# wildltr/ptranking

Measured on NVIDIA H100. Metric: queries/sec (LambdaRank train step, 256-doc lists), higher is better.
Workload: dtype f32

## Files before the change

ptranking_b200/csrc/ffnet_tc.cuh:

```cuda
#pragma once
#include "common.cuh"
#include "tc.cuh"
#include "ffnet_act.cuh"

namespace ptrb200 {

struct RowsGemmArgs {
    const float* P;
    const float* scale;
    const float* shift;
    int act;
    int gr_prev;
    DropCfg drop;
    const float* P2;
    const float *kc1, *kc3, *kc0;
    int gr_cur;
    const unsigned char* b_img_hi;
    const unsigned char* b_img_lo;
    const float* bias;
    float* a_out;
    float* Out;
    double* partials;
    int rows, K, N, NP;
    int n_tile;
// ... 558 lines not shown
    #pragma unroll
                    for (int i = 0; i < RW_PU; ++i) { cur[i] = pre[i]; cur2[i] = pre2[i]; }
                    if (q + 1 < total_q) {
                        if (c + 1 < nchunks) fetch(c + 1); else { point(it + 1); fetch(0); }
                    }
                    if (q >= 2) tc::mbar_wait(afree + s, ((q - 2) >> 1) & 1);
                    unsigned char* a_hi = a_ring + s * 32768;
                    if (partial && c == lastc) {
    #pragma unroll
                        for (int i = 0; i < RW_PU; ++i) {
                            const int jB = jB_[i];
                            if (jB < zfill) {
                                float4 v = make_float4(0.f, 0.f, 0.f, 0.f);
                                if (jB < vlast && rB < nrows) {
                                    const int col = lastc * 32 + jB * 4;
                                    const size_t e0 = (size_t)(row0 + rB) * K + col;
                                    const size_t co = (per_group ? (size_t)((row0 + rB) / g.gr_prev) * K : (size_t)0) + col;
                                    const size_t kc = ((fused_dz && g.gr_cur < g.rows) ? (size_t)((row0 + rB) / g.gr_cur) * K : (size_t)0) + col;
                                    v = xform(cur[i], cur2[i], has_coef ? g.scale + co : nullptr, has_coef ? g.shift + co : nullptr, kc,
                                              (uint64_t)e0 >> 2, (MODE == RG_FWD && g.a_out) ? g.a_out + e0 : nullptr);
                                }
                                store_split(a_hi, a_hi + 16384, tc::swz_offset(rB, jB), v, PASSES == 3, PASSES == 1 && g.round_bf16 != 0);
                            }
                        }
                    } else {
                        const bool kv = c * 32 + j4 < K;
    #pragma unroll
                        for (int i = 0; i < RW_PU; ++i) {
                            float4 v = make_float4(0.f, 0.f, 0.f, 0.f);
                            if (live[i] && kv)
                                v = xform(cur[i], cur2[i], has_coef ? sc[i] + c * 32 : nullptr, has_coef ? sh[i] + c * 32 : nullptr,
                                          kco[i] + c * 32, dq[i] + c * 8, aout[i] ? aout[i] + c * 32 : nullptr);
                            store_split(a_hi, a_hi + 16384, sw_[i], v, PASSES == 3, PASSES == 1 && g.round_bf16 != 0);
                        }
                    }
                    tc::fence_proxy_async();
                    __syncwarp();
                    if (lane == 0) tc::mbar_arrive(aready + s);
                }
            }
        }
    } else {
        tc::setmaxnreg_dec<RW_CONS_REGS>();
        if (my_tiles > 0) {
        const int wg = warp >> 2;
        if (tid == 0) {
            tc::mbar_expect_tx(wfull, (uint32_t)(nchunks * wchunk * (PASSES == 3 ? 2 : 1)));
            for (int c = 0; c < nchunks; ++c) {
                tc::bulk_g2s(w_hi + (size_t)c * wchunk, g.b_img_hi + (size_t)c * wchunk, wchunk, wfull);
                if (PASSES == 3) tc::bulk_g2s(w_lo + (size_t)c * wchunk, g.b_img_lo + (size_t)c * wchunk, wchunk, wfull);
            }
        }
        tc::mbar_wait(wfull, 0);
        const uint32_t a_base = tc::smem_u32(a_ring) + wg * 8192, wh_base = tc::smem_u32(w_hi), wl_base = tc::smem_u32(w_lo);
        double acc1 = 0.0, acc2 = 0.0;
        tc::with_width(NP, [&](auto W) {
        constexpr int NPc = decltype(W)::value;
        int q = 0;
        for (int it = 0; it < my_tiles; ++it) {
            const int t = blockIdx.x + it * gridDim.x;
            int row0, nrows;
            rw_tile(g, t, row0, nrows);
            float acc[NPc / 2];
#pragma unroll
            for (int e = 0; e < NPc / 2; ++e) acc[e] = 0.0f;
    #pragma unroll (KT ? 8 : 1)
            for (int c = 0; c < nchunks; ++c, ++q) {
                const int s = q & 1;
                tc::mbar_wait(aready + s, (q >> 1) & 1);
                uint32_t a_addr = a_base + s * 32768, b_off = c * wchunk;
                asm volatile("" : "+r"(a_addr), "+r"(b_off));
                const uint64_t ah = tc::smem_desc_sw128(a_addr, 1024), al = tc::smem_desc_sw128(a_addr + 16384, 1024);
                const uint64_t bh = tc::smem_desc_sw128(wh_base + b_off, 1024), bl = tc::smem_desc_sw128(wl_base + b_off, 1024);
                tc::wg_fence();
#pragma unroll
                for (int st = 0; st < 4; ++st) {
                    if (PASSES == 3) {
                        tc::mma_tf32<NPc>(acc, al + 2 * st, bh + 2 * st, 1u);
                        tc::mma_tf32<NPc>(acc, ah + 2 * st, bl + 2 * st, 1u);
                    }
                    tc::mma_tf32<NPc>(acc, ah + 2 * st, bh + 2 * st, 1u);
                }
                tc::wg_commit();
                tc::wg_wait<1>();
                if (c > 0) { __syncwarp(); if (lane == 0) tc::mbar_arrive(afree + (s ^ 1)); }
            }
            tc::wg_wait<0>();
            __syncwarp();
            if (lane == 0) tc::mbar_arrive(afree + ((q - 1) & 1));
            const float* bias = g.bias;
            asm volatile("" : "+l"(bias));
            bool live[2];
            float* orow[2];
#pragma unroll
            for (int h = 0; h < 2; ++h) {
                const int r = wg * 64 + tc::acc_row(2 * h);
                live[h] = r < nrows;
                orow[h] = g.Out + (size_t)(row0 + min(r, nrows - 1)) * N;
            }
            if (MODE == RG_FWD) {
#pragma unroll
                for (int e = 0; e < NPc / 2; ++e) {
                    const int col = tc::acc_col(e);
                    if (col >= N) { acc[e] = 0.0f; continue; }
                    acc[e] += __ldg(bias + col);
                }
            } else if (g.drop.thr && (N & 3) == 0) {
                const bool odd = lane & 1;
#pragma unroll
                for (int e = 0; e < NPc / 2; e += 4) {
                    const int col = tc::acc_col(e);
                    const uint64_t el = (uint64_t)(row0 + wg * 64 + tc::acc_row(e) + (odd ? 8 : 0)) * N + (col & ~3);
                    const uint64_t d = dropout_draw4(g.drop.key, el >> 2);
                    const uint32_t other = __shfl_xor_sync(0xffffffffu, odd ? (uint32_t)d : (uint32_t)(d >> 32), 1);
                    const uint32_t ur = odd ? other : (uint32_t)d;
                    const uint32_t ur8 = odd ? (uint32_t)(d >> 32) : other;
                    if (col >= N) { acc[e] = acc[e + 1] = acc[e + 2] = acc[e + 3] = 0.0f; continue; }
                    acc[e] = (ur & 0xffffu) >= g.drop.thr ? acc[e] * g.drop.scale : 0.0f;
                    acc[e + 1] = (ur >> 16) >= g.drop.thr ? acc[e + 1] * g.drop.scale : 0.0f;
                    acc[e + 2] = (ur8 & 0xffffu) >= g.drop.thr ? acc[e + 2] * g.drop.scale : 0.0f;
                    acc[e + 3] = (ur8 >> 16) >= g.drop.thr ? acc[e + 3] * g.drop.scale : 0.0f;
                }
            } else {
#pragma unroll
                for (int e = 0; e < NPc / 2; ++e) {
                    const int col = tc::acc_col(e);
                    if (col >= N) { acc[e] = 0.0f; continue; }
                    if (g.drop.thr) {
                        const int r = wg * 64 + tc::acc_row(e);
                        acc[e] = dropout_keep(g.drop.key, (uint64_t)(row0 + r) * N + col, g.drop.thr) ? acc[e] * g.drop.scale : 0.0f;
                    }
                }
            }
#pragma unroll
            for (int e = 0; e < NPc / 2; e += 2) {
                const int col = tc::acc_col(e), h = (e >> 1) & 1;
                if (!live[h] || col >= N) continue;
                if ((N & 1) == 0) *reinterpret_cast<float2*>(orow[h] + col) = make_float2(acc[e], acc[e + 1]);
                else { orow[h][col] = acc[e]; if (col + 1 < N) orow[h][col + 1] = acc[e + 1]; }
            }
            if (MODE == RG_FWD && x.stats_mode) {
                int sl = lane, sw = warp;
                asm volatile("" : "+r"(sl), "+r"(sw));
#pragma unroll
                for (int j = 0; j < NPc / 16; ++j) {
                    const float* w = acc + 8 * j;
                    float s[8];
#pragma unroll
                    for (int p = 0; p < 4; ++p) {
                        const int e0 = (p >> 1) * 4 + (p & 1), e1 = e0 + 2;
                        const float v0 = live[0] ? w[e0] : 0.0f, v1 = live[1] ? w[e1] : 0.0f;
                        s[p] = v0 + v1; s[4 + p] = v0 * v0 + v1 * v1;
                    }
#pragma unroll
                    for (int st = 0; st < 3; ++st) {
                        const int h = 4 >> st, o = 4 << st;
                        const bool up = sl & o;
#pragma unroll
                        for (int i = 0; i < h; ++i) {
                            float keep = s[i], send = s[i + h];
                            if (up) { const float t = keep; keep = send; send = t; }
                            s[i] = keep + __shfl_xor_sync(0xffffffffu, send, o);
                        }
                    }
                    const int v = ((sl >> 2) & 1) * 4 + ((sl >> 3) & 1) * 2 + ((sl >> 4) & 1), p = v & 3;
                    const int col = j * 16 + (p >> 1) * 8 + 2 * (sl & 3) + (p & 1);
                    stat_sm[(sw * NP + col) * 2 + (v >> 2)] = s[0];
                }
                asm volatile("bar.sync 2, 256;" ::: "memory");
                if (tid < N) {
                    double s1 = 0.0, s2 = 0.0;
#pragma unroll
                    for (int w = 0; w < RW_EPI_WARPS; ++w) { s1 += (double)stat_sm[(w * NP + tid) * 2]; s2 += (double)stat_sm[(w * NP + tid) * 2 + 1]; }
                    if (x.stats_mode == 2) {
                        double* p = g.partials + ((size_t)t * N + tid) * 2;
                        p[0] = s1; p[1] = s2;
                    } else { acc1 += s1; acc2 += s2; }
                }
                asm volatile("bar.sync 2, 256;" ::: "memory");
            }
        }
        });
        if (MODE == RG_FWD && x.stats_mode == 1 && tid < N) {
            double* p = g.partials + ((size_t)blockIdx.x * N + tid) * 2;
            p[0] = acc1; p[1] = acc2;
        }
        } else if (MODE == RG_FWD && x.stats_mode == 1 && tid < N) {
            double* p = g.partials + ((size_t)blockIdx.x * N + tid) * 2;
            p[0] = 0.0; p[1] = 0.0;
        }
    }
}

struct WgradArgs {
    const float* Z2;
    const float *kc1, *kc3, *kc0;
    int gr_cur;
    const float* dZ;
    const float* P;
    const float* scale;
    const float* shift;
    int act, gr_prev;
    DropCfg drop;
    float* partials;
    int rows, K, N;
    int KP;
    int N_full, K_full;
    int kb;
    int tile_rows;
    int stages;
    int round_bf16;
};

constexpr int WG_THREADS = 512;
constexpr int WG_MAX_STAGES = 4;

template <int PASSES, bool XB = false>
__global__ void __launch_bounds__(WG_THREADS, 1) wgrad_tc_kernel(WgradArgs g) {
    extern __shared__ __align__(1024) unsigned char smem_raw[];
    unsigned char* base = reinterpret_cast<unsigned char*>((reinterpret_cast<uintptr_t>(smem_raw) + 1023) & ~(uintptr_t)1023);
    const int R = g.tile_rows;
    const int m0 = blockIdx.y * 128, kk0 = blockIdx.z * g.kb;
    const int N = min(128, g.N_full - m0), K = min(g.kb, g.K_full - kk0), KP = ((K + 15) / 16) * 16;
    const int Nmax = min(128, g.N_full), Kmax = min(g.kb, g.K_full);
    const bool blocked = gridDim.y > 1 || gridDim.z > 1;
    const int KPmax = ((Kmax + 15) / 16) * 16;
    const int zop_bytes = 128 * 128, pop_bytes = KPmax * 128;
    const int op_bytes = (zop_bytes + pop_bytes) * (PASSES == 3 ? 2 : 1);
    const bool fused_dz = g.Z2 != nullptr;
    const int rawz1 = ((R * Nmax * 4 + 127) / 128) * 128;
    constexpr int PB = XB ? 2 : 4;
    const int rawz_bytes = rawz1 * (fused_dz ? 2 : 1), rawp_bytes = ((R * Kmax * PB + 127) / 128) * 128;
    const int stages = g.stages;
    unsigned char* opbuf = base;
    unsigned char* rawbuf = opbuf + 2 * op_bytes;
    unsigned char* tail = rawbuf + stages * (rawz_bytes + rawp_bytes);
    uint64_t* full = reinterpret_cast<uint64_t*>(tail);

    const int tid = threadIdx.x, warp = tid >> 5, lane = tid & 31, wg = warp >> 2;
    if (tid == 0) {
        for (int s = 0; s < stages; ++s) tc::mbar_init(full + s, 1);
        tc::mbar_fence_init();
    }
    const int ntiles = (g.rows + R - 1) / R;
    const int my_tiles = blockIdx.x < ntiles ? (ntiles - blockIdx.x + gridDim.x - 1) / gridDim.x : 0;

    bool p_bulk_ok = true;
    if constexpr (XB) p_bulk_ok = ((reinterpret_cast<uintptr_t>(g.P) & 15) == 0) && (!blocked || (K % 8 == 0 && g.K_full % 8 == 0));
    auto p_bulk = [&](int nrows) -> bool {
        if constexpr (XB) return p_bulk_ok && (blocked || (((uint32_t)nrows * K * 2) & 15) == 0);
        else return true;
    };

    auto issue_load = [&](int it, int s) {
        const int t = blockIdx.x + it * gridDim.x;
        const int row0 = t * R, nrows = min(R, g.rows - row0);
        const bool pbk = p_bulk(nrows);
        const uint32_t zb = (uint32_t)nrows * N * 4, pb = pbk ? (uint32_t)nrows * K * PB : 0u;
        unsigned char* rz = rawbuf + s * (rawz_bytes + rawp_bytes);
        if (!blocked) {
            if (lane == 0) {
                if ((zb & 15) == 0) {
                    tc::mbar_expect_tx(full + s, (fused_dz ? 2 * zb : zb) + pb);
                    tc::bulk_g2s(rz, g.dZ + (size_t)row0 * N, zb, full + s);
                    if (fused_dz) tc::bulk_g2s(rz + rawz1, g.Z2 + (size_t)row0 * N, zb, full + s);
                } else {
                    tc::mbar_expect_tx(full + s, pb);
                }
                if constexpr (XB) { if (pbk) tc::bulk_g2s(rz + rawz_bytes, reinterpret_cast<const uint16_t*>(g.P) + (size_t)row0 * K, pb, full + s); }
                else tc::bulk_g2s(rz + rawz_bytes, g.P + (size_t)row0 * K, pb, full + s);
            }
        } else {
            const bool z_bulk = (N & 3) == 0;
            if (lane == 0) tc::mbar_expect_tx(full + s, (z_bulk ? zb : 0u) + pb);
            __syncwarp();
            if (lane < nrows) {
                if (z_bulk) tc::bulk_g2s(rz + (size_t)lane * N * 4, g.dZ + (size_t)(row0 + lane) * g.N_full + m0, (uint32_t)N * 4, full + s);
                if constexpr (XB) {
                    if (pbk) tc::bulk_g2s(rz + rawz_bytes + (size_t)lane * K * 2, reinterpret_cast<const uint16_t*>(g.P) + (size_t)(row0 + lane) * g.K_full + kk0,
                                          (uint32_t)K * 2, full + s);
                } else tc::bulk_g2s(rz + rawz_bytes + (size_t)lane * K * 4, g.P + (size_t)(row0 + lane) * g.K_full + kk0, (uint32_t)K * 4, full + s);
            }
            __syncwarp();
        }
    };

    const bool plain_p = !g.scale && g.act == PTRB200_AF_NONE && !g.drop.thr;
    const bool single_group = fused_dz && g.gr_cur >= g.rows;
    float* coef = reinterpret_cast<float*>(tail + 128);
    {
        const uint32_t op_s = tc::smem_u32(opbuf);
        for (int e = tid; e < 2 * op_bytes / 16; e += WG_THREADS) tc::sts128(op_s + (uint32_t)e * 16u, make_float4(0.f, 0.f, 0.f, 0.f));
        if (single_group)
            for (int e = tid; e < 3 * 128; e += WG_THREADS) {
                const int which = e >> 7, n = e & 127;
                const float* src = which == 0 ? g.kc1 : which == 1 ? g.kc3 : g.kc0;
                coef[e] = n < N ? __ldg(src + m0 + n) : 0.0f;
            }
        __syncthreads();
    }
    if (warp == 0)
        for (int it = 0; it < min(stages, my_tiles); ++it) issue_load(it, it);

    auto put = [&](unsigned char* hi, unsigned char* lo, uint32_t off, float4 v) {
        if (PASSES == 3) {
            float4 h, l;
            tc::split_tf32(v.x, h.x, l.x); tc::split_tf32(v.y, h.y, l.y); tc::split_tf32(v.z, h.z, l.z); tc::split_tf32(v.w, h.w, l.w);
            *reinterpret_cast<float4*>(hi + off) = h;
            *reinterpret_cast<float4*>(lo + off) = l;
        } else {
            if (g.round_bf16) v = make_float4(bf16_rn(v.x), bf16_rn(v.y), bf16_rn(v.z), bf16_rn(v.w));
            *reinterpret_cast<float4*>(hi + off) = v;
        }
    };
    const int mh = wg & 1, KPh = ((KP / 16 + 1) / 2) * 16, c0 = (wg >> 1) ? KP - KPh : 0, cw0 = (wg >> 1) ? KPh : 0;
    const int RQ = R / 4;

    tc::with_width(KPh, [&](auto W) {
    constexpr int NPc = decltype(W)::value;
    float acc[NPc / 2];
#pragma unroll
    for (int e = 0; e < NPc / 2; ++e) acc[e] = 0.0f;
    for (int it = 0; it < my_tiles; ++it) {
        const int t = blockIdx.x + it * gridDim.x, o = it & 1, s = it % stages;
        const int row0 = t * R, nrows = min(R, g.rows - row0);
        const float* rz = reinterpret_cast<const float*>(rawbuf + s * (rawz_bytes + rawp_bytes));
        const float* rp = reinterpret_cast<const float*>(rawbuf + s * (rawz_bytes + rawp_bytes) + rawz_bytes);
        if (blocked ? (N & 3) != 0 : (((uint32_t)nrows * N * 4) & 15) != 0) {
            float* rzw = const_cast<float*>(rz);
            for (int e = tid; e < nrows * N; e += WG_THREADS) rzw[e] = g.dZ[(size_t)(row0 + e / N) * g.N_full + m0 + e % N];
            __syncthreads();
        }
        if constexpr (XB) {
            if (!p_bulk(nrows)) {
                uint16_t* rpw = reinterpret_cast<uint16_t*>(rawbuf + s * (rawz_bytes + rawp_bytes) + rawz_bytes);
                const uint16_t* src = reinterpret_cast<const uint16_t*>(g.P);
                for (int e = tid; e < nrows * K; e += WG_THREADS) rpw[e] = src[(size_t)(row0 + e / K) * g.K_full + kk0 + e % K];
                __syncthreads();
            }
        }
        tc::mbar_wait(full + s, (it / stages) & 1);
        unsigned char* zh = opbuf + o * op_bytes;
        unsigned char* zl = zh + zop_bytes;
        unsigned char* ph = zh + (PASSES == 3 ? 2 : 1) * zop_bytes;
        unsigned char* pl = ph + pop_bytes;
        for (int u = tid; u < 128 * RQ; u += WG_THREADS) {
            const int n = u & 127, qq = u >> 7;
            if (n >= N) continue;
            float v[4];
            const size_t grp_off_base = (size_t)m0 + n;
#pragma unroll
            for (int e = 0; e < 4; ++e) {
                const int r = qq * 4 + e;
                float x = 0.0f;
                if (r < nrows) {
                    x = rz[r * N + n];
                    if (fused_dz) {
                        const float z = rz[rawz1 / 4 + r * N + n];
                        float a1, a3, a0;
                        if (single_group) { a1 = coef[n]; a3 = coef[128 + n]; a0 = coef[256 + n]; }
                        else {
                            const size_t go = (size_t)((row0 + r) / g.gr_cur) * g.N_full + grp_off_base;
                            a1 = __ldg(g.kc1 + go); a3 = __ldg(g.kc3 + go); a0 = __ldg(g.kc0 + go);
                        }
                        x = fmaf(a1, x, fmaf(a3, z, a0));
                    }
                }
                v[e] = x;
            }
            put(zh, zl, tc::swz_offset(n, qq), make_float4(v[0], v[1], v[2], v[3]));
        }
        for (int u = tid; u < KP * RQ; u += WG_THREADS) {
            const int k = u % KP, qq = u / KP;
            if (k >= K) continue;
            float v[4];
#pragma unroll
            for (int e = 0; e < 4; ++e) {
                const int r = qq * 4 + e;
                float x = 0.0f;
                if (r < nrows) {
                    if constexpr (XB) x = __uint_as_float((uint32_t)reinterpret_cast<const uint16_t*>(rp)[r * K + k] << 16);
                    else x = rp[r * K + k];
                    if (!plain_p) {
                        const int row = row0 + r, col = kk0 + k;
                        if (g.scale) {
                            const size_t co = (g.gr_prev < g.rows ? (size_t)(row / g.gr_prev) * g.K_full : 0) + col;
                            x = fmaf(x, __ldg(g.scale + co), __ldg(g.shift + co));
                        }
                        if (g.act != PTRB200_AF_NONE) x = activate(g.act, x).y;
                        if (g.drop.thr) x = dropout_keep(g.drop.key, (uint64_t)row * g.K_full + col, g.drop.thr) ? x * g.drop.scale : 0.0f;
                    }
                }
                v[e] = x;
            }
            put(ph, pl, tc::swz_offset(k, qq), make_float4(v[0], v[1], v[2], v[3]));
        }
        tc::fence_proxy_async();
        __syncthreads();
        if (warp == 0 && it + stages < my_tiles) issue_load(it + stages, s);
        const uint32_t a_s = tc::smem_u32(zh) + mh * 8192, b_s = tc::smem_u32(ph) + c0 * 128;
        const uint64_t ah = tc::smem_desc_sw128(a_s, 1024), bh = tc::smem_desc_sw128(b_s, 1024);
        const uint64_t al = tc::smem_desc_sw128(a_s + zop_bytes, 1024), bl = tc::smem_desc_sw128(b_s + pop_bytes, 1024);
        tc::wg_fence();
#pragma unroll
        for (int st = 0; st < 4; ++st) {
            if (PASSES == 3) {
                tc::mma_tf32<NPc>(acc, al + 2 * st, bh + 2 * st, 1u);
                tc::mma_tf32<NPc>(acc, ah + 2 * st, bl + 2 * st, 1u);
            }
            tc::mma_tf32<NPc>(acc, ah + 2 * st, bh + 2 * st, 1u);
        }
        tc::wg_commit();
        tc::wg_wait<0>();
    }
    float* dst = g.partials + (size_t)blockIdx.x * g.N_full * g.K_full + (size_t)m0 * g.K_full + kk0;
#pragma unroll
    for (int e = 0; e < NPc / 2; ++e) {
        const int n = mh * 64 + tc::acc_row(e), k = c0 + tc::acc_col(e);
        if (n < N && k >= cw0 && k < K) dst[(size_t)n * g.K_full + k] = acc[e];
    }
    });
}

}
```

ptranking_b200/csrc/tc.cuh:

```cuda
#pragma once
#include <cuda_runtime.h>
#include <stdint.h>

namespace ptrb200 {
namespace tc {

template <int N> struct WidthT { static constexpr int value = N; };

constexpr int CHUNK_BYTES = 128;
constexpr int ATOM_BYTES = 1024;

__device__ __forceinline__ uint32_t smem_u32(const void* p) { return (uint32_t)__cvta_generic_to_shared(p); }

__device__ __forceinline__ uint32_t swz_offset(int r, int j) {
    return (uint32_t)((r >> 3) * ATOM_BYTES + (r & 7) * CHUNK_BYTES + ((j ^ (r & 7)) << 4));
}

__device__ __forceinline__ float4 lds128(uint32_t addr) {
    float4 v;
    asm volatile("ld.shared.v4.f32 {%0,%1,%2,%3}, [%4];" : "=f"(v.x), "=f"(v.y), "=f"(v.z), "=f"(v.w) : "r"(addr) : "memory");
    return v;
}
__device__ __forceinline__ float lds32(uint32_t addr) {
    float v;
    asm volatile("ld.shared.f32 %0, [%1];" : "=f"(v) : "r"(addr) : "memory");
    return v;
}
__device__ __forceinline__ void sts128(uint32_t addr, float4 v) {
    asm volatile("st.shared.v4.f32 [%0], {%1,%2,%3,%4};" ::"r"(addr), "f"(v.x), "f"(v.y), "f"(v.z), "f"(v.w) : "memory");
}

__device__ __forceinline__ void mbar_init(uint64_t* bar, uint32_t count) {
    asm volatile("mbarrier.init.shared::cta.b64 [%0], %1;" ::"r"(smem_u32(bar)), "r"(count) : "memory");
}
__device__ __forceinline__ void mbar_fence_init() { asm volatile("fence.mbarrier_init.release.cluster;" ::: "memory"); }
__device__ __forceinline__ void mbar_arrive(uint64_t* bar) {
    asm volatile("{\n\t.reg .b64 st;\n\tmbarrier.arrive.shared::cta.b64 st, [%0];\n\t}" ::"r"(smem_u32(bar)) : "memory");
}
__device__ __forceinline__ void mbar_expect_tx(uint64_t* bar, uint32_t bytes) {
    asm volatile("{\n\t.reg .b64 st;\n\tmbarrier.arrive.expect_tx.shared::cta.b64 st, [%0], %1;\n\t}" ::"r"(smem_u32(bar)), "r"(bytes) : "memory");
}
__device__ __forceinline__ bool mbar_try_wait(uint64_t* bar, uint32_t parity) {
    uint32_t ok;
    asm volatile(
        "{\n\t.reg .pred p;\n\t"
        "mbarrier.try_wait.parity.shared::cta.b64 p, [%1], %2;\n\t"
        "selp.u32 %0, 1, 0, p;\n\t}"
        : "=r"(ok) : "r"(smem_u32(bar)), "r"(parity) : "memory");
    return ok != 0;
}
__device__ __forceinline__ void mbar_wait(uint64_t* bar, uint32_t parity) {
    while (!mbar_try_wait(bar, parity)) {}
}
__device__ __forceinline__ void mbar_wait_relaxed(uint64_t* bar, uint32_t parity) {
    while (!mbar_try_wait(bar, parity)) { __nanosleep(40); }
}
__device__ __forceinline__ void fence_proxy_async() { asm volatile("fence.proxy.async.shared::cta;" ::: "memory"); }

template <int N>
__device__ __forceinline__ void setmaxnreg_dec() { asm volatile("setmaxnreg.dec.sync.aligned.u32 %0;" ::"n"(N)); }
template <int N>
__device__ __forceinline__ void setmaxnreg_inc() { asm volatile("setmaxnreg.inc.sync.aligned.u32 %0;" ::"n"(N)); }

__device__ __forceinline__ void bulk_g2s(void* smem_dst, const void* gmem_src, uint32_t bytes, uint64_t* bar) {
    asm volatile("cp.async.bulk.shared::cluster.global.mbarrier::complete_tx::bytes [%0], [%1], %2, [%3];"
                 ::"r"(smem_u32(smem_dst)), "l"(gmem_src), "r"(bytes), "r"(smem_u32(bar)) : "memory");
}
__device__ __forceinline__ void bulk_s2g(void* gmem_dst, const void* smem_src, uint32_t bytes) {
    asm volatile("cp.async.bulk.global.shared::cta.bulk_group [%0], [%1], %2;"
                 ::"l"(gmem_dst), "r"(smem_u32(smem_src)), "r"(bytes) : "memory");
}
__device__ __forceinline__ void bulk_commit() { asm volatile("cp.async.bulk.commit_group;" ::: "memory"); }
template <int N>
__device__ __forceinline__ void bulk_wait_read() { asm volatile("cp.async.bulk.wait_group.read %0;" ::"n"(N) : "memory"); }
template <int N>
__device__ __forceinline__ void bulk_wait() { asm volatile("cp.async.bulk.wait_group %0;" ::"n"(N) : "memory"); }

__device__ __forceinline__ uint64_t smem_desc_sw128(uint32_t smem_addr, uint32_t sbo_bytes) {
    uint64_t d = 0;
    d |= (uint64_t)((smem_addr & 0x3ffffu) >> 4);
    d |= (uint64_t)1 << 16;
    d |= (uint64_t)((sbo_bytes >> 4) & 0x3fffu) << 32;
    d |= (uint64_t)1 << 62;
    return d;
}

__device__ __forceinline__ void wg_fence() { asm volatile("wgmma.fence.sync.aligned;" ::: "memory"); }
__device__ __forceinline__ void wg_commit() { asm volatile("wgmma.commit_group.sync.aligned;" ::: "memory"); }
template <int N>
__device__ __forceinline__ void wg_wait() { asm volatile("wgmma.wait_group.sync.aligned %0;" ::"n"(N) : "memory"); }

template <int N>
__device__ __forceinline__ void mma_tf32(float (&d)[N / 2], uint64_t a_desc, uint64_t b_desc, uint32_t scale_d);

template <>
__device__ __forceinline__ void mma_tf32<16>(float (&d)[8], uint64_t a_desc, uint64_t b_desc, uint32_t scale_d) {
    asm volatile(
        "{\n\t.reg .pred p;\n\tsetp.ne.b32 p, %10, 0;\n\t"
        "wgmma.mma_async.sync.aligned.m64n16k8.f32.tf32.tf32 {%0,%1,%2,%3,%4,%5,%6,%7}, %8, %9, p, 1, 1;\n\t}"
        : "+f"(d[0]), "+f"(d[1]), "+f"(d[2]), "+f"(d[3]), "+f"(d[4]), "+f"(d[5]), "+f"(d[6]), "+f"(d[7])
        : "l"(a_desc), "l"(b_desc), "r"(scale_d) : "memory");
}

template <>
__device__ __forceinline__ void mma_tf32<32>(float (&d)[16], uint64_t a_desc, uint64_t b_desc, uint32_t scale_d) {
    asm volatile(
        "{\n\t.reg .pred p;\n\tsetp.ne.b32 p, %18, 0;\n\t"
        "wgmma.mma_async.sync.aligned.m64n32k8.f32.tf32.tf32 {%0,%1,%2,%3,%4,%5,%6,%7,%8,%9,%10,%11,%12,%13,%14,%15}, %16, %17, p, 1, 1;\n\t}"
        : "+f"(d[0]), "+f"(d[1]), "+f"(d[2]), "+f"(d[3]), "+f"(d[4]), "+f"(d[5]), "+f"(d[6]), "+f"(d[7]), "+f"(d[8]), "+f"(d[9]), "+f"(d[10]), "+f"(d[11]), "+f"(d[12]), "+f"(d[13]), "+f"(d[14]), "+f"(d[15])
        : "l"(a_desc), "l"(b_desc), "r"(scale_d) : "memory");
}

template <>
__device__ __forceinline__ void mma_tf32<48>(float (&d)[24], uint64_t a_desc, uint64_t b_desc, uint32_t scale_d) {
    asm volatile(
        "{\n\t.reg .pred p;\n\tsetp.ne.b32 p, %26, 0;\n\t"
        "wgmma.mma_async.sync.aligned.m64n48k8.f32.tf32.tf32 {%0,%1,%2,%3,%4,%5,%6,%7,%8,%9,%10,%11,%12,%13,%14,%15,%16,%17,%18,%19,%20,%21,%22,%23}, %24, %25, p, 1, 1;\n\t}"
        : "+f"(d[0]), "+f"(d[1]), "+f"(d[2]), "+f"(d[3]), "+f"(d[4]), "+f"(d[5]), "+f"(d[6]), "+f"(d[7]), "+f"(d[8]), "+f"(d[9]), "+f"(d[10]), "+f"(d[11]), "+f"(d[12]), "+f"(d[13]), "+f"(d[14]), "+f"(d[15]), "+f"(d[16]), "+f"(d[17]), "+f"(d[18]), "+f"(d[19]), "+f"(d[20]), "+f"(d[21]), "+f"(d[22]), "+f"(d[23])
        : "l"(a_desc), "l"(b_desc), "r"(scale_d) : "memory");
}

template <>
__device__ __forceinline__ void mma_tf32<64>(float (&d)[32], uint64_t a_desc, uint64_t b_desc, uint32_t scale_d) {
    asm volatile(
        "{\n\t.reg .pred p;\n\tsetp.ne.b32 p, %34, 0;\n\t"
        "wgmma.mma_async.sync.aligned.m64n64k8.f32.tf32.tf32 {%0,%1,%2,%3,%4,%5,%6,%7,%8,%9,%10,%11,%12,%13,%14,%15,%16,%17,%18,%19,%20,%21,%22,%23,%24,%25,%26,%27,%28,%29,%30,%31}, %32, %33, p, 1, 1;\n\t}"
        : "+f"(d[0]), "+f"(d[1]), "+f"(d[2]), "+f"(d[3]), "+f"(d[4]), "+f"(d[5]), "+f"(d[6]), "+f"(d[7]), "+f"(d[8]), "+f"(d[9]), "+f"(d[10]), "+f"(d[11]), "+f"(d[12]), "+f"(d[13]), "+f"(d[14]), "+f"(d[15]), "+f"(d[16]), "+f"(d[17]), "+f"(d[18]), "+f"(d[19]), "+f"(d[20]), "+f"(d[21]), "+f"(d[22]), "+f"(d[23]), "+f"(d[24]), "+f"(d[25]), "+f"(d[26]), "+f"(d[27]), "+f"(d[28]), "+f"(d[29]), "+f"(d[30]), "+f"(d[31])
        : "l"(a_desc), "l"(b_desc), "r"(scale_d) : "memory");
}

template <>
__device__ __forceinline__ void mma_tf32<80>(float (&d)[40], uint64_t a_desc, uint64_t b_desc, uint32_t scale_d) {
    asm volatile(
        "{\n\t.reg .pred p;\n\tsetp.ne.b32 p, %42, 0;\n\t"
        "wgmma.mma_async.sync.aligned.m64n80k8.f32.tf32.tf32 {%0,%1,%2,%3,%4,%5,%6,%7,%8,%9,%10,%11,%12,%13,%14,%15,%16,%17,%18,%19,%20,%21,%22,%23,%24,%25,%26,%27,%28,%29,%30,%31,%32,%33,%34,%35,%36,%37,%38,%39}, %40, %41, p, 1, 1;\n\t}"
        : "+f"(d[0]), "+f"(d[1]), "+f"(d[2]), "+f"(d[3]), "+f"(d[4]), "+f"(d[5]), "+f"(d[6]), "+f"(d[7]), "+f"(d[8]), "+f"(d[9]), "+f"(d[10]), "+f"(d[11]), "+f"(d[12]), "+f"(d[13]), "+f"(d[14]), "+f"(d[15]), "+f"(d[16]), "+f"(d[17]), "+f"(d[18]), "+f"(d[19]), "+f"(d[20]), "+f"(d[21]), "+f"(d[22]), "+f"(d[23]), "+f"(d[24]), "+f"(d[25]), "+f"(d[26]), "+f"(d[27]), "+f"(d[28]), "+f"(d[29]), "+f"(d[30]), "+f"(d[31]), "+f"(d[32]), "+f"(d[33]), "+f"(d[34]), "+f"(d[35]), "+f"(d[36]), "+f"(d[37]), "+f"(d[38]), "+f"(d[39])
        : "l"(a_desc), "l"(b_desc), "r"(scale_d) : "memory");
}

template <>
__device__ __forceinline__ void mma_tf32<96>(float (&d)[48], uint64_t a_desc, uint64_t b_desc, uint32_t scale_d) {
    asm volatile(
        "{\n\t.reg .pred p;\n\tsetp.ne.b32 p, %50, 0;\n\t"
        "wgmma.mma_async.sync.aligned.m64n96k8.f32.tf32.tf32 {%0,%1,%2,%3,%4,%5,%6,%7,%8,%9,%10,%11,%12,%13,%14,%15,%16,%17,%18,%19,%20,%21,%22,%23,%24,%25,%26,%27,%28,%29,%30,%31,%32,%33,%34,%35,%36,%37,%38,%39,%40,%41,%42,%43,%44,%45,%46,%47}, %48, %49, p, 1, 1;\n\t}"
        : "+f"(d[0]), "+f"(d[1]), "+f"(d[2]), "+f"(d[3]), "+f"(d[4]), "+f"(d[5]), "+f"(d[6]), "+f"(d[7]), "+f"(d[8]), "+f"(d[9]), "+f"(d[10]), "+f"(d[11]), "+f"(d[12]), "+f"(d[13]), "+f"(d[14]), "+f"(d[15]), "+f"(d[16]), "+f"(d[17]), "+f"(d[18]), "+f"(d[19]), "+f"(d[20]), "+f"(d[21]), "+f"(d[22]), "+f"(d[23]), "+f"(d[24]), "+f"(d[25]), "+f"(d[26]), "+f"(d[27]), "+f"(d[28]), "+f"(d[29]), "+f"(d[30]), "+f"(d[31]), "+f"(d[32]), "+f"(d[33]), "+f"(d[34]), "+f"(d[35]), "+f"(d[36]), "+f"(d[37]), "+f"(d[38]), "+f"(d[39]), "+f"(d[40]), "+f"(d[41]), "+f"(d[42]), "+f"(d[43]), "+f"(d[44]), "+f"(d[45]), "+f"(d[46]), "+f"(d[47])
        : "l"(a_desc), "l"(b_desc), "r"(scale_d) : "memory");
}

template <>
__device__ __forceinline__ void mma_tf32<112>(float (&d)[56], uint64_t a_desc, uint64_t b_desc, uint32_t scale_d) {
    asm volatile(
        "{\n\t.reg .pred p;\n\tsetp.ne.b32 p, %58, 0;\n\t"
        "wgmma.mma_async.sync.aligned.m64n112k8.f32.tf32.tf32 {%0,%1,%2,%3,%4,%5,%6,%7,%8,%9,%10,%11,%12,%13,%14,%15,%16,%17,%18,%19,%20,%21,%22,%23,%24,%25,%26,%27,%28,%29,%30,%31,%32,%33,%34,%35,%36,%37,%38,%39,%40,%41,%42,%43,%44,%45,%46,%47,%48,%49,%50,%51,%52,%53,%54,%55}, %56, %57, p, 1, 1;\n\t}"
        : "+f"(d[0]), "+f"(d[1]), "+f"(d[2]), "+f"(d[3]), "+f"(d[4]), "+f"(d[5]), "+f"(d[6]), "+f"(d[7]), "+f"(d[8]), "+f"(d[9]), "+f"(d[10]), "+f"(d[11]), "+f"(d[12]), "+f"(d[13]), "+f"(d[14]), "+f"(d[15]), "+f"(d[16]), "+f"(d[17]), "+f"(d[18]), "+f"(d[19]), "+f"(d[20]), "+f"(d[21]), "+f"(d[22]), "+f"(d[23]), "+f"(d[24]), "+f"(d[25]), "+f"(d[26]), "+f"(d[27]), "+f"(d[28]), "+f"(d[29]), "+f"(d[30]), "+f"(d[31]), "+f"(d[32]), "+f"(d[33]), "+f"(d[34]), "+f"(d[35]), "+f"(d[36]), "+f"(d[37]), "+f"(d[38]), "+f"(d[39]), "+f"(d[40]), "+f"(d[41]), "+f"(d[42]), "+f"(d[43]), "+f"(d[44]), "+f"(d[45]), "+f"(d[46]), "+f"(d[47]), "+f"(d[48]), "+f"(d[49]), "+f"(d[50]), "+f"(d[51]), "+f"(d[52]), "+f"(d[53]), "+f"(d[54]), "+f"(d[55])
        : "l"(a_desc), "l"(b_desc), "r"(scale_d) : "memory");
}

template <>
__device__ __forceinline__ void mma_tf32<128>(float (&d)[64], uint64_t a_desc, uint64_t b_desc, uint32_t scale_d) {
    asm volatile(
        "{\n\t.reg .pred p;\n\tsetp.ne.b32 p, %66, 0;\n\t"
        "wgmma.mma_async.sync.aligned.m64n128k8.f32.tf32.tf32 {%0,%1,%2,%3,%4,%5,%6,%7,%8,%9,%10,%11,%12,%13,%14,%15,%16,%17,%18,%19,%20,%21,%22,%23,%24,%25,%26,%27,%28,%29,%30,%31,%32,%33,%34,%35,%36,%37,%38,%39,%40,%41,%42,%43,%44,%45,%46,%47,%48,%49,%50,%51,%52,%53,%54,%55,%56,%57,%58,%59,%60,%61,%62,%63}, %64, %65, p, 1, 1;\n\t}"
        : "+f"(d[0]), "+f"(d[1]), "+f"(d[2]), "+f"(d[3]), "+f"(d[4]), "+f"(d[5]), "+f"(d[6]), "+f"(d[7]), "+f"(d[8]), "+f"(d[9]), "+f"(d[10]), "+f"(d[11]), "+f"(d[12]), "+f"(d[13]), "+f"(d[14]), "+f"(d[15]), "+f"(d[16]), "+f"(d[17]), "+f"(d[18]), "+f"(d[19]), "+f"(d[20]), "+f"(d[21]), "+f"(d[22]), "+f"(d[23]), "+f"(d[24]), "+f"(d[25]), "+f"(d[26]), "+f"(d[27]), "+f"(d[28]), "+f"(d[29]), "+f"(d[30]), "+f"(d[31]), "+f"(d[32]), "+f"(d[33]), "+f"(d[34]), "+f"(d[35]), "+f"(d[36]), "+f"(d[37]), "+f"(d[38]), "+f"(d[39]), "+f"(d[40]), "+f"(d[41]), "+f"(d[42]), "+f"(d[43]), "+f"(d[44]), "+f"(d[45]), "+f"(d[46]), "+f"(d[47]), "+f"(d[48]), "+f"(d[49]), "+f"(d[50]), "+f"(d[51]), "+f"(d[52]), "+f"(d[53]), "+f"(d[54]), "+f"(d[55]), "+f"(d[56]), "+f"(d[57]), "+f"(d[58]), "+f"(d[59]), "+f"(d[60]), "+f"(d[61]), "+f"(d[62]), "+f"(d[63])
        : "l"(a_desc), "l"(b_desc), "r"(scale_d) : "memory");
}

__device__ __forceinline__ int acc_row(int e) { return 16 * ((threadIdx.x >> 5) & 3) + ((threadIdx.x & 31) >> 2) + 8 * ((e >> 1) & 1); }
__device__ __forceinline__ int acc_col(int e) { return 8 * (e >> 2) + 2 * (threadIdx.x & 3) + (e & 1); }

template <typename F>
__device__ __forceinline__ void with_width(int np, F&& f) {
    switch (np) {
        case 16: f(WidthT<16>{}); break;
        case 32: f(WidthT<32>{}); break;
        case 48: f(WidthT<48>{}); break;
        case 64: f(WidthT<64>{}); break;
        case 80: f(WidthT<80>{}); break;
        case 96: f(WidthT<96>{}); break;
        case 112: f(WidthT<112>{}); break;
        default: f(WidthT<128>{}); break;
    }
}

__device__ __forceinline__ uint32_t swz_elem(int r, int k) { return swz_offset(r, k >> 2) + (uint32_t)((k & 3) << 2); }

__device__ __forceinline__ void split_tf32(float x, float& hi, float& lo) {
    hi = __uint_as_float(__float_as_uint(x) & 0xffffe000u);
    lo = x - hi;
}

__device__ __forceinline__ void split_tf32_rn(float x, float& hi, float& lo) {
    hi = __uint_as_float((__float_as_uint(x) + 0x1000u) & 0xffffe000u);
    const float r = x - hi;
    lo = __uint_as_float((__float_as_uint(r) + 0x1000u) & 0xffffe000u);
}

}
}
```

Measured before the change: 235,300.

## Defer wgmma wait to overlap tensor-core MMA with next tile's operand staging

The wgmma wait moves from right after each tile's commit to just before the next tile's barrier. The asynchronous MMA on one operand buffer now runs while threads convert and swizzle the next tile into the other double buffer. Shared-memory accesses switch to explicit 32-bit shared addresses (lds32/lds_u16/sts128), which should avoid generic-address conversion. Empty asm register fences keep the compiler from touching accumulators while wgmma is in flight. The risk is correctness if the buffer reuse distance or the fences are wrong.

```diff
diff --git a/ptranking_b200/csrc/ffnet_tc.cuh b/ptranking_b200/csrc/ffnet_tc.cuh
--- a/ptranking_b200/csrc/ffnet_tc.cuh
+++ b/ptranking_b200/csrc/ffnet_tc.cuh
@@ -884,17 +884,18 @@
     if (warp == 0)
         for (int it = 0; it < min(stages, my_tiles); ++it) issue_load(it, it);
 
-    auto put = [&](unsigned char* hi, unsigned char* lo, uint32_t off, float4 v) {
+    auto put = [&](uint32_t hi, uint32_t lo, uint32_t off, float4 v) {
         if (PASSES == 3) {
             float4 h, l;
             tc::split_tf32(v.x, h.x, l.x); tc::split_tf32(v.y, h.y, l.y); tc::split_tf32(v.z, h.z, l.z); tc::split_tf32(v.w, h.w, l.w);
-            *reinterpret_cast<float4*>(hi + off) = h;
-            *reinterpret_cast<float4*>(lo + off) = l;
+            tc::sts128(hi + off, h);
+            tc::sts128(lo + off, l);
         } else {
             if (g.round_bf16) v = make_float4(bf16_rn(v.x), bf16_rn(v.y), bf16_rn(v.z), bf16_rn(v.w));
-            *reinterpret_cast<float4*>(hi + off) = v;
+            tc::sts128(hi + off, v);
         }
     };
+    const uint32_t raw_s = tc::smem_u32(rawbuf), op_s0 = tc::smem_u32(opbuf), coef_s = tc::smem_u32(coef);
     const int mh = wg & 1, KPh = ((KP / 16 + 1) / 2) * 16, c0 = (wg >> 1) ? KP - KPh : 0, cw0 = (wg >> 1) ? KPh : 0;
     const int RQ = R / 4;
 
@@ -903,11 +904,11 @@
     float acc[NPc / 2];
 #pragma unroll
     for (int e = 0; e < NPc / 2; ++e) acc[e] = 0.0f;
+    tc::fence_acc(acc);
     for (int it = 0; it < my_tiles; ++it) {
         const int t = blockIdx.x + it * gridDim.x, o = it & 1, s = it % stages;
         const int row0 = t * R, nrows = min(R, g.rows - row0);
         const float* rz = reinterpret_cast<const float*>(rawbuf + s * (rawz_bytes + rawp_bytes));
-        const float* rp = reinterpret_cast<const float*>(rawbuf + s * (rawz_bytes + rawp_bytes) + rawz_bytes);
         if (blocked ? (N & 3) != 0 : (((uint32_t)nrows * N * 4) & 15) != 0) {
             float* rzw = const_cast<float*>(rz);
             for (int e = tid; e < nrows * N; e += WG_THREADS) rzw[e] = g.dZ[(size_t)(row0 + e / N) * g.N_full + m0 + e % N];
@@ -922,10 +923,9 @@
             }
         }
         tc::mbar_wait(full + s, (it / stages) & 1);
-        unsigned char* zh = opbuf + o * op_bytes;
-        unsigned char* zl = zh + zop_bytes;
-        unsigned char* ph = zh + (PASSES == 3 ? 2 : 1) * zop_bytes;
-        unsigned char* pl = ph + pop_bytes;
+        const uint32_t zh = op_s0 + o * op_bytes, zl = zh + zop_bytes;
+        const uint32_t ph = zh + (PASSES == 3 ? 2 : 1) * zop_bytes, pl = ph + pop_bytes;
+        const uint32_t rz_s = raw_s + s * (rawz_bytes + rawp_bytes), rp_s = rz_s + rawz_bytes;
         for (int u = tid; u < 128 * RQ; u += WG_THREADS) {
             const int n = u & 127, qq = u >> 7;
             if (n >= N) continue;
@@ -936,11 +936,13 @@
                 const int r = qq * 4 + e;
                 float x = 0.0f;
                 if (r < nrows) {
-                    x = rz[r * N + n];
+                    x = tc::lds32(rz_s + (uint32_t)(r * N + n) * 4u);
                     if (fused_dz) {
-                        const float z = rz[rawz1 / 4 + r * N + n];
+                        const float z = tc::lds32(rz_s + rawz1 + (uint32_t)(r * N + n) * 4u);
                         float a1, a3, a0;
-                        if (single_group) { a1 = coef[n]; a3 = coef[128 + n]; a0 = coef[256 + n]; }
+                        if (single_group) {
+                            a1 = tc::lds32(coef_s + n * 4u); a3 = tc::lds32(coef_s + (128 + n) * 4u); a0 = tc::lds32(coef_s + (256 + n) * 4u);
+                        }
                         else {
                             const size_t go = (size_t)((row0 + r) / g.gr_cur) * g.N_full + grp_off_base;
                             a1 = __ldg(g.kc1 + go); a3 = __ldg(g.kc3 + go); a0 = __ldg(g.kc0 + go);
@@ -961,8 +963,8 @@
                 const int r = qq * 4 + e;
                 float x = 0.0f;
                 if (r < nrows) {
-                    if constexpr (XB) x = __uint_as_float((uint32_t)reinterpret_cast<const uint16_t*>(rp)[r * K + k] << 16);
-                    else x = rp[r * K + k];
+                    if constexpr (XB) x = __uint_as_float(tc::lds_u16(rp_s + (uint32_t)(r * K + k) * 2u) << 16);
+                    else x = tc::lds32(rp_s + (uint32_t)(r * K + k) * 4u);
                     if (!plain_p) {
                         const int row = row0 + r, col = kk0 + k;
                         if (g.scale) {
@@ -978,11 +980,14 @@
             put(ph, pl, tc::swz_offset(k, qq), make_float4(v[0], v[1], v[2], v[3]));
         }
         tc::fence_proxy_async();
+        tc::wg_wait<0>();
+        tc::fence_acc(acc);
         __syncthreads();
         if (warp == 0 && it + stages < my_tiles) issue_load(it + stages, s);
-        const uint32_t a_s = tc::smem_u32(zh) + mh * 8192, b_s = tc::smem_u32(ph) + c0 * 128;
+        const uint32_t a_s = zh + mh * 8192, b_s = ph + c0 * 128;
         const uint64_t ah = tc::smem_desc_sw128(a_s, 1024), bh = tc::smem_desc_sw128(b_s, 1024);
         const uint64_t al = tc::smem_desc_sw128(a_s + zop_bytes, 1024), bl = tc::smem_desc_sw128(b_s + pop_bytes, 1024);
+        tc::fence_acc(acc);
         tc::wg_fence();
 #pragma unroll
         for (int st = 0; st < 4; ++st) {
@@ -993,8 +998,9 @@
             tc::mma_tf32<NPc>(acc, ah + 2 * st, bh + 2 * st, 1u);
         }
         tc::wg_commit();
-        tc::wg_wait<0>();
-    }
+    }
+    tc::wg_wait<0>();
+    tc::fence_acc(acc);
     float* dst = g.partials + (size_t)blockIdx.x * g.N_full * g.K_full + (size_t)m0 * g.K_full + kk0;
 #pragma unroll
     for (int e = 0; e < NPc / 2; ++e) {
diff --git a/ptranking_b200/csrc/tc.cuh b/ptranking_b200/csrc/tc.cuh
--- a/ptranking_b200/csrc/tc.cuh
+++ b/ptranking_b200/csrc/tc.cuh
@@ -24,6 +24,11 @@
 __device__ __forceinline__ float lds32(uint32_t addr) {
     float v;
     asm volatile("ld.shared.f32 %0, [%1];" : "=f"(v) : "r"(addr) : "memory");
+    return v;
+}
+__device__ __forceinline__ uint32_t lds_u16(uint32_t addr) {
+    unsigned short v;
+    asm volatile("ld.shared.u16 %0, [%1];" : "=h"(v) : "r"(addr) : "memory");
     return v;
 }
 __device__ __forceinline__ void sts128(uint32_t addr, float4 v) {
@@ -89,6 +94,11 @@
 __device__ __forceinline__ void wg_commit() { asm volatile("wgmma.commit_group.sync.aligned;" ::: "memory"); }
 template <int N>
 __device__ __forceinline__ void wg_wait() { asm volatile("wgmma.wait_group.sync.aligned %0;" ::"n"(N) : "memory"); }
+template <int M>
+__device__ __forceinline__ void fence_acc(float (&d)[M]) {
+#pragma unroll
+    for (int i = 0; i < M; ++i) asm volatile("" : "+f"(d[i])::"memory");
+}
 
 template <int N>
 __device__ __forceinline__ void mma_tf32(float (&d)[N / 2], uint64_t a_desc, uint64_t b_desc, uint32_t scale_d);
```

Result: faster. 242,900 (median of 6 runs) (+3.2%).
